# treangenlab/bronko

Measured on AMD Instinct MI355X. Metric: reads/sec through call k-mer->pileup, SARS-CoV-2 k=21, higher is better.
Workload: dtype u64

## Files before the change

### bronko_amd/csrc/bk_engine.cpp

```cpp
#include <hip/hip_runtime.h>

#include <algorithm>
#include <cstdarg>
#include <cstdio>
#include <cstdlib>
#include <cstring>
#include <memory>
#include <string>
#include <vector>

#include "../host/lcb.hpp"
#include "bk_engine.h"

thread_local std::string g_err;

int fail(int code, const char* fmt, ...) {
    char buf[1024];
    va_list ap;
    va_start(ap, fmt);
    vsnprintf(buf, sizeof buf, fmt, ap);
    va_end(ap);
    g_err = buf;
    return code;
}
// ... 430 lines not shown
        int share = ix.n_cus - ix.n_cus / 4;
        if (const char* fr = test_env("BK_ITEM_SHARE")) share = std::max(1, std::min(ix.n_cus, ix.n_cus * atoi(fr) / 16));
        grid = bk::items_grid(take, ix.family.load() > 1 ? share : ix.n_cus);
        if (const char* gr = test_env("BK_ITEM_GRID")) grid = std::max<uint32_t>(1, std::min<uint32_t>(grid, (uint32_t)atoi(gr)));
    }
    return take;
}
static int make_l2_room(bk_engine* e, bk::ScanArgs& a, uint64_t l2_cap) {
    if (e->l2_bits.n < a.n_records * a.l2_words || e->l2_diag.n < a.n_records) {
        BK_HIP(hipStreamSynchronize(e->stream));
        const uint64_t recs = std::min<uint64_t>(std::max<uint64_t>(a.n_records + a.n_records / 4, 1 << 16), l2_cap);
        BK_HIP(e->l2_bits.alloc((size_t)recs * a.l2_words)); BK_HIP(e->n_bits.alloc((size_t)recs * a.l2_words)); BK_HIP(e->l2_diag.alloc((size_t)recs));
        BK_HIP(e->l2_any.alloc((size_t)(recs + 31) / 32)); BK_HIP(e->n_any.alloc((size_t)(recs + 31) / 32));
        for (DevBuf<unsigned int>* b : {&e->l2_bits, &e->l2_any, &e->n_bits, &e->n_any}) BK_HIP(hipMemsetAsync(b->p, 0, b->n * sizeof(unsigned int), e->stream));
    }
    a.l2_bits = e->l2_bits.p; a.l2_diag = e->l2_diag.p; a.l2_any = e->l2_any.p; a.n_bits = e->n_bits.p; a.n_any = e->n_any.p;
    return BK_OK;
}
static int bin_items(bk_engine* e, bk::ScanArgs& a, int mate, uint32_t grid, bool wait_v) {
    const IndexTables& ix = *e->ix;
    MatePlane& pl = e->mate[mate];
    bk_engine::Span sp(e, 3);
    bk::BinArgs b{};
    b.ig = e->ig; b.items = e->items.p; b.tab = e->item_tab.p; b.gext = e->item_gext.p; b.n_wg = grid; b.ov = e->ov.p; b.ov_n = e->ov_n.p; b.ov_cap = (uint32_t)e->ov.n;
    b.ov_par = e->ov_par; e->ov_par ^= 1u;
    b.id_at = ix.id_at.p; b.cell_codes = ix.cell_codes.p + bk::scan_ref_pad_words(); b.win_lo = a.win_lo; b.win_dev = a.win_dev; b.total_cells = (uint32_t)ix.total_cells;
    b.counters = pl.counters.p; b.v_off = ix.v_off; b.v_real_len = bk::v_real_len(ix.n_full, ix.v_span); b.rl = (uint32_t)ix.v_span + 1u;
    const bool v_clean = pl.take_v_clean();
    b.v_mode = ix.item_v_mode >= 0 ? ix.item_v_mode : (v_clean ? 2 : 1);
    if (const char* ba = test_env("BK_BIN_ABLATE")) b.ablate = atoi(ba);
    if (wait_v) {
        e->pending.on = true; e->pending.mate = mate; e->pending.b = b;
        b.part = 1;
        a.touch_v = pl.fuse_touch.p; a.rl_recip = ~0ull / (unsigned long long)(ix.v_span + 1) + 1ull;
        pl.items_wait();
    } else {
        pl.no_more_waiting();
        if (e->fuse_ok) a.touch_v = nullptr;
    }
    BK_HIP(bk::launch_bin_count(b, e->stream));
    return BK_OK;
}
static int level2_and_fold(bk_engine* e, const bk::ScanArgs& a, int mate, uint32_t grid) {
    const IndexTables& ix = *e->ix;
    bk_engine::Span sp(e, 3);
    if (int rc = l2_count_report(e, a)) return rc;
    if (ix.ablate == 1 || ix.ablate == 4) {
        BK_HIP(hipMemsetAsync(e->n_bits.p, 0, (size_t)a.n_records * a.l2_words * sizeof(unsigned int), e->stream));
        BK_HIP(hipMemsetAsync(e->n_any.p, 0, e->n_any.n * sizeof(unsigned int), e->stream));
    }
    else BK_HIP(bk::launch_level2(a, ix.n_cus, e->stream));
    if (!e->use_items) {
        bk::FoldArgs f{};
        f.slabs = e->slabs.p; f.n_slabs = grid; f.n_lds_bins = ix.n_lds_bins; f.id_at = ix.id_at.p; f.cell_codes = ix.cell_codes.p + bk::scan_ref_pad_words(); f.win_lo = a.win_lo; f.win_dev = a.win_dev; f.touch_e = a.touch_e;
        f.counters = e->mate[mate].counters.p;
        bk::launch_fold(f, e->stream);
    }
    return BK_OK;
}
static int push_device(bk_engine* e, int mate, const uint32_t* d_words, uint32_t stride_words, const uint16_t* d_lens, uint64_t n,
                       const unsigned long long* n_records_dev = nullptr, uint64_t kmers_upper = 0) {
    MatePlane& pl = e->mate[mate];
    if (int rc = pl.zero_if_stale(e)) return rc;
    const uint64_t upper = kmers_upper ? kmers_upper : n * (uint64_t)stride_words * 16;
    if (int rc = ensure_ktab_room(e, upper)) return rc;
    if (e->dump) { if (int rc = dump_push(e, mate, d_words, stride_words, d_lens, n, n_records_dev, upper)) return rc; }
    pl.written();
    if (int rc = l2_stats_arm(e)) return rc;
    bk::ScanArgs a = scan_args(e, mate, d_words, stride_words, d_lens, n, n_records_dev);
    if (e->ix->W <= 0) {
        bk::launch_count_kmers(a, e->stream);
    } else {
        if (int rc = choose_window(e, a, n)) return rc;
        const uint64_t l2_cap = std::max<uint64_t>(64, ((1ull << 30) / sizeof(unsigned int)) / a.l2_words);
        for (uint64_t base = 0; base < n; base += a.n_records) {
            uint32_t grid = 0;
            a.rec_base = base; a.n_records = next_launch(e, n - base, l2_cap, grid);
            if (int rc = make_l2_room(e, a, l2_cap)) return rc;
            if (int rc = flush_pending_items(e)) return rc;
            const bool wait_v = e->fuse_ok && a.n_direct && !pl.fuse_off && e->ix->item_v_mode < 0;
            a.l2_plan = e->use_items && e->ix->n_files == 1 && e->ix->family.load() >= 4 && !test_env("BK_NO_L2_PLAN") ? e->l2_plan.p : nullptr;
            {
                bk_engine::Span sp(e, 0);
                if (e->use_items) { a.ov_par = e->ov_par; BK_HIP(bk::launch_scan_items(a, grid, e->stream)); }
                else BK_HIP(bk::launch_scan_count(a, grid, e->stream));
            }
            if (e->use_items) { if (int rc = bin_items(e, a, mate, grid, wait_v)) return rc; }
            if (int rc = level2_and_fold(e, a, mate, grid)) return rc;
        }
    }
    BK_HIP(hipGetLastError());
    if (!n_records_dev) pl.pushed_records += n;
    return note_ktab_fill(e);
}

static constexpr int kPush = 1;
static int push_checks(bk_engine* e, int mate, uint64_t n, bool batch_ok, const char* bad_batch, bool too_large) {
    if (!e) return fail(BK_ERR_INVALID, "null engine");
    if (!e->in_sample) return fail(BK_ERR_STATE, "bk_push_reads_* called before bk_sample_begin");
    if (mate < 0 || mate > 1) return fail(BK_ERR_INVALID, "mate must be 0 or 1");
    if (n == 0) return BK_OK;
    if (!batch_ok) return fail(BK_ERR_INVALID, "%s", bad_batch);
    if (too_large) return fail(BK_ERR_INVALID, "batch too large: push at most 2^32 bases per call");
    BK_HIP(hipSetDevice(e->device));
    return kPush;
}
static int packed_checks(bk_engine* e, int mate, const void* words, uint32_t stride_words, const void* lens, uint64_t n) {
    return push_checks(e, mate, n, words && lens && stride_words != 0 && stride_words <= 4096, "bad record batch",
                       stride_words != 0 && n > (1ull << 32) / ((uint64_t)stride_words * 16));
}
struct PackGeom {
    uint32_t stride; uint64_t cap;
    PackGeom(int k, uint64_t n_reads, uint64_t total, uint64_t longest)
        : stride((uint32_t)std::min<uint64_t>((std::max<uint64_t>(longest, (uint64_t)k) + 15) / 16, 4095)),
          cap(n_reads + total / (uint64_t)k + total / (std::min<uint64_t>((uint64_t)stride * 16, 65535) - (uint64_t)(k - 1)) + 16) {}
};
static int pack_and_push(bk_engine* e, int mate, bk_engine::IngestSlot& sl, const uint8_t* bases, uint32_t shift, const unsigned long long* offsets,
                         uint64_t n_reads, uint64_t total, PackGeom g, const bk::QualArgs* q = nullptr) {
    bk::PackArgs pa{};
    pa.shift = shift; pa.bases = bases; pa.offsets = offsets; pa.n_reads = n_reads; pa.k = e->ix->k; pa.stride_words = g.stride;
    pa.words = sl.d_words.p; pa.lens = sl.d_lens.p; pa.cap = g.cap; pa.n_records = sl.d_nrec.p; pa.work = sl.d_work.p;
    { bk_engine::Span sp(e, 2); bk::launch_pack_reads(pa, e->kstats.p + mate * 4 + 0, e->stream, q); }
    return push_device(e, mate, sl.d_words.p, g.stride, sl.d_lens.p, g.cap, sl.d_nrec.p, total);
}

static constexpr int kMaxMinQual = 93;

static int push_ascii(bk_engine* e, int mate, const uint8_t* buf, const uint8_t* qual, const uint64_t* offsets, uint64_t n_reads, uint32_t thr) {
    const bool too_large = buf && offsets && n_reads && offsets[n_reads] - offsets[0] >= (1ull << 32);
    if (int rc = push_checks(e, mate, n_reads, buf && offsets, "bad read batch", too_large); rc != kPush) return rc;
    const uint64_t base0 = offsets[0], total = offsets[n_reads] - base0;
    if (!e->copy_stream) BK_HIP(hipStreamCreateWithFlags(&e->copy_stream, hipStreamNonBlocking));
    bk_engine::IngestSlot& sl = e->slots[e->next_slot];
    e->next_slot = (e->next_slot + 1) % 3;
    if (!sl.done) { BK_HIP(hipEventCreateWithFlags(&sl.done, hipEventDisableTiming)); BK_HIP(hipEventCreateWithFlags(&sl.uploaded, hipEventDisableTiming)); }
    if (sl.busy) { BK_HIP(hipEventSynchronize(sl.done)); sl.busy = false; }

    if (sl.h_bases_cap < total + 1) {
        if (sl.h_bases) BK_HIP(hipHostFree(sl.h_bases));
        sl.h_bases_cap = total + total / 4 + 4096;
        BK_HIP(hipHostMalloc(reinterpret_cast<void**>(&sl.h_bases), sl.h_bases_cap, hipHostMallocDefault));
    }
    if (sl.h_off_cap < n_reads + 1) {
        if (sl.h_off) BK_HIP(hipHostFree(sl.h_off));
        sl.h_off_cap = n_reads + n_reads / 4 + 1024;
        BK_HIP(hipHostMalloc(reinterpret_cast<void**>(&sl.h_off), sl.h_off_cap * sizeof(unsigned long long), hipHostMallocDefault));
    }
    if (qual && sl.h_quals_cap < total + 1) {
        if (sl.h_quals) BK_HIP(hipHostFree(sl.h_quals));
        sl.h_quals_cap = total + total / 4 + 4096;
        BK_HIP(hipHostMalloc(reinterpret_cast<void**>(&sl.h_quals), sl.h_quals_cap, hipHostMallocDefault));
    }
    std::memcpy(sl.h_bases, buf + base0, total);
    if (qual) std::memcpy(sl.h_quals, qual + base0, total);
    uint64_t longest = 0;
    for (uint64_t i = 0; i <= n_reads; i++) {
        sl.h_off[i] = offsets[i] - base0;
        if (i) longest = std::max(longest, offsets[i] - offsets[i - 1]);
    }
    const PackGeom g(e->ix->k, n_reads, total, longest);

    if (sl.d_bases.n < total + 1) BK_HIP(sl.d_bases.alloc(total + total / 4 + 4096));
    if (qual && sl.d_quals.n < total + 1) BK_HIP(sl.d_quals.alloc(total + total / 4 + 4096));
    if (sl.d_off.n < n_reads + 1) BK_HIP(sl.d_off.alloc(n_reads + n_reads / 4 + 1024));
    if (sl.d_words.n < g.cap * g.stride) BK_HIP(sl.d_words.alloc(g.cap * g.stride + g.cap * g.stride / 4));
    if (sl.d_lens.n < g.cap) BK_HIP(sl.d_lens.alloc(g.cap + g.cap / 4));
    if (!sl.d_nrec.p) BK_HIP(sl.d_nrec.alloc(4));
// ... 725 lines not shown
```

### bronko_amd/csrc/bk_kernels.h

```cpp
#pragma once
#include <hip/hip_runtime.h>

#include "../../include/bronko_hip.h"
#include "bk_device.h"

namespace bk {

struct ItemGeom {
    uint32_t n_ebins, n_vbins;
    uint32_t cap_e, cap_v;
    uint32_t vq_log2;
    uint32_t wg_items;
    uint32_t wg_stride;
    uint32_t grid_max;
};
constexpr uint32_t kEBinLog2 = 7;
constexpr uint32_t kERunMax = 255;
constexpr uint32_t kEBinSpan = (1u << kEBinLog2) + kERunMax;
constexpr uint32_t kItemGCap = 256;

struct ScanArgs {
    const IndexView* ixp;
    int32_t k, wstart, W, v_omin, v_span;
    uint64_t v_off;
    uint32_t total_cells, n_u;
    const uint32_t* ref_words;
    const uint32_t* cell_codes;
    const uint32_t* cell_has;
    const uint32_t* cell_clean;
    const uint32_t* cell_clean3;
    const uint32_t* cell_yf;
    const uint32_t* cell_yr;
    const uint32_t* id_at;
    const uint32_t* cell_fast;
    const uint2* cell_blk;
    const uint32_t* cell_nat;
    const uint32_t* cell_natrow;
    const uint2* seed_tab;
    uint32_t seed_log2;
    const uint2* seed_tab2;
    uint32_t seed2_log2;
    const uint32_t* rc_words;
    const uint32_t* words;
    const uint16_t* lens;
    uint64_t rec_base;
    uint64_t n_records;
    const unsigned long long* n_records_dev;
    uint32_t stride_words;
    unsigned long long* counters;
    unsigned int* slabs;
    unsigned int* n_bits;
    unsigned int* n_any;
    unsigned int* l2_bits;
    unsigned int* l2_any;
    unsigned int* l2_plan;
    uint32_t l2_min_grid;
    uint2* l2_diag;
    uint32_t l2_words;
    uint32_t n_lds_bins;
    uint32_t win_lo;
    const uint32_t* win_dev;
    const uint32_t* occ;
    int32_t win_file, n_files;
    int ref_in_lds;
    unsigned long long* kmer_total;
    unsigned long long* ktab_keys;
    unsigned int* ktab_cnt;
    uint32_t ktab_log2;
    unsigned long long* ktab_overflow;
    uint32_t mate;
    unsigned int* touch_v;
    unsigned int* touch_b;
    unsigned int* touch_p;
    unsigned int* touch_e;
    unsigned long long rl_recip;
    ItemGeom ig;
    unsigned short* items;
    unsigned short* tab;
    unsigned short* gext;
    unsigned int* ov;
    unsigned long long* ov_n;
    uint32_t ov_cap;
    uint32_t ov_par;
    int n_direct;
    uint32_t stage_off;
    int ablate;
    unsigned long long* dbg;
};

struct FinalizeArgs {
    IndexView ix;
    const unsigned long long* counters;
    uint64_t elem_lo, elem_hi;
    unsigned long long ci, cs, cx;
    unsigned long long* pileup;
    size_t plane;
    unsigned long long* stats;
    unsigned char* present;
    unsigned long long* kept_total;
    unsigned long long* distinct_total;
    unsigned int* partials;
    int row_exact, row_general;
    const uint32_t* file_cell_lo;
    uint32_t max_file_cells;
    unsigned int* deferred;
    unsigned long long* deferred_n;
    int clear_v;
    unsigned int* deferred_mask;
    unsigned int* n_deferred;
    unsigned long long* ktab_keys;
    unsigned int* ktab_cnt;
    uint32_t ktab_log2;
    unsigned long long* ktab_overflow;
    uint32_t mate;
    const unsigned int* v_list;
    const unsigned int* p_list;
    const unsigned int* e_list;
    const unsigned int* n_list;
    int mode;
    const int* sel;
    int sel_file;
    unsigned int* lean_e_list;
    unsigned int* lean_n_list;
    int no_lean;
    const unsigned int* tail_e_list;
    const unsigned int* tail_n_list;
    unsigned long long* zero_e;
    size_t zero_e_n;
    int gather;
    int gather_ablate;
    unsigned long long* alias_hits;
    unsigned int* n_alias_hits;
    unsigned int alias_cap;
    const uint64_t* merged_slots;
    uint32_t n_merged_slots;
    const unsigned short* f_items;
    const unsigned short* f_tab;
    const unsigned short* f_gext;
    const unsigned int* f_ov;
    const unsigned long long* f_ov_n;
    uint32_t f_ov_cap, f_ov_par, f_n_wg;
    ItemGeom f_ig;
    unsigned int* f_touch;
};

struct FoldArgs {
    const unsigned int* slabs;
    uint32_t n_slabs;
    uint32_t n_lds_bins;
    const uint32_t* id_at;
    uint32_t win_lo;
    const uint32_t* win_dev;
    unsigned int* touch_e;
    const uint32_t* cell_codes;
    unsigned long long* counters;
};

struct PackArgs {
    const uint8_t* bases;
    uint32_t shift;
    const unsigned long long* offsets;
    uint64_t n_reads;
    int32_t k;
    uint32_t stride_words;
    uint32_t* words;
    uint16_t* lens;
    uint64_t cap;
// ... 145 lines not shown
```

### bronko_amd/csrc/bk_scan_items.hip

```cpp
#include <hip/hip_runtime.h>

#include <algorithm>
#include <mutex>
#include <utility>
#include <vector>

#include "bk_device.h"
#include "bk_kernels.h"
#include "bk_scan_common.h"

namespace bk {

constexpr int kItemBlock = 1024;
constexpr int kItemWaves = kItemBlock / 64;
constexpr int kItemGroupsPerCu = 1;
constexpr uint32_t kListCap = 256;
constexpr uint32_t kListWords = kListCap + 4u;
constexpr uint32_t kDealRing = 32;
constexpr size_t kItemLdsFixed = (4 + 4 + 2 * kDealRing + kItemWaves * kListWords) * sizeof(unsigned int);
constexpr int kBinBlock = 256;
constexpr uint32_t kMaxChunkMismatches = 24;
constexpr uint32_t kStageMaxWords = 12;

__device__ __forceinline__ void item_direct(const __attribute__((address_space(4))) ScanArgs* ap, uint32_t bin, uint32_t item, uint32_t win_lo) {
    const __attribute__((address_space(4))) ScanArgs& a = *ap;
    if (bin < a.ig.n_ebins) {
        const uint32_t c0 = win_lo + (bin << kEBinLog2) + (item & 127u), n = ((item >> 7) & 255u) + 1u, rev = item >> 15;
        for (uint32_t i = 0; i < n; ++i) {
            const uint32_t cell = c0 + i;
            const uint32_t id = a.id_at[cell];
            const uint32_t rc = ((a.cell_codes[kRefPadWords + (cell >> 4)] >> (2u * (cell & 15u))) & 3u) == 2u ? 1u : 0u;
            atomicAdd(a.counters + 2 * (size_t)id + (rc ^ rev), 1ull);
        }
    } else {
        const uint64_t at = (uint64_t)(bin - a.ig.n_ebins) * ((6ull << a.ig.vq_log2) * (uint32_t)(a.v_span + 1)) + (item & 0x7fffu);
        atomicAdd(a.counters + a.v_off + at, (item & 0x8000u) ? ~0ull : 1ull);
    }
}

template <int KT, bool STAGED>
__global__ __launch_bounds__(kItemBlock) void scan_items_kernel(ScanArgs a) {
    extern __shared__ __attribute__((aligned(16))) unsigned char smem[];
    unsigned int* block_kmers = reinterpret_cast<unsigned int*>(smem);
    unsigned int* wg_ctr = block_kmers + 4;
    uint2* ring = reinterpret_cast<uint2*>(wg_ctr + 4);
    unsigned int* lst_all = wg_ctr + 4 + 2 * kDealRing;
    unsigned int* cnt = lst_all + kItemWaves * kListWords;
    const uint32_t n_eb = a.ig.n_ebins, n_bins = n_eb + a.ig.n_vbins, cap_e = a.ig.cap_e, cap_v = a.ig.cap_v;
    const uint32_t nb_pad = (n_bins + 3u) & ~3u;
    unsigned short* buck = reinterpret_cast<unsigned short*>(cnt + nb_pad);
    unsigned int* lds_ref = reinterpret_cast<unsigned int*>(smem + ((kItemLdsFixed + (size_t)nb_pad * 4u + (size_t)a.ig.wg_stride * 2u + 7u) & ~(size_t)7u));

    const int lane = threadIdx.x & 63;
    const int wave = __builtin_amdgcn_readfirstlane((int)(threadIdx.x >> 6));
    unsigned int* const lst = lst_all + (uint32_t)wave * kListWords;
    typedef const __attribute__((address_space(4))) ScanArgs* ColdArgs;
    const ColdArgs cold0 = (ColdArgs)__builtin_amdgcn_kernarg_segment_ptr();
    auto cold = [&]() __attribute__((always_inline)) -> ColdArgs { ColdArgs p = cold0; asm volatile("" : "+s"(p)); return p; };

    asm volatile("v_mov_b32 v127, 0" ::: "v127");
    BK_DBG_CLOCK(a, 0);
    const uint32_t total = a.total_cells;
    const uint32_t win_lo = a.win_dev ? a.win_dev[1] : a.win_lo;
    const uint32_t win_file = a.win_dev ? a.win_dev[0] : (uint32_t)a.win_file;
    const uint32_t lds_cells = min(total - win_lo, a.n_lds_bins);
    const uint32_t n_refw = kRefPadWords + (lds_cells + 15) / 16 + kRefBackWords;
    const uint32_t n_bitw = kBitPadWords + (lds_cells + 31) / 32 + kBitBackWords;
    const uint32_t n_blk = (lds_cells + 63) / 64 + 2;
    const uint32_t blk_w0 = (n_refw + 2u * n_bitw + 1u) & ~1u;
    const uint32_t rc_lo = total - win_lo - lds_cells, rc_base = rc_lo & 15u;
    const uint32_t rc_w0 = blk_w0 + 2u * n_blk;
    uint64_t n_records = a.n_records;
    if (a.n_records_dev) {
        const uint64_t nd = *a.n_records_dev;
        n_records = nd > a.rec_base ? min(nd - a.rec_base, a.n_records) : 0ull;
    }
    const uint32_t* const words0 = a.words + a.rec_base * a.stride_words;
    const uint16_t* const lens0 = a.lens + a.rec_base;
    const uint64_t n_tiles = (n_records + 63) / 64;
    unsigned int* const deal_ctr = reinterpret_cast<unsigned int*>(cold()->ov_n + 2);
    const uint64_t t_hi = n_tiles;
    const uint32_t sw = a.stride_words;
    unsigned int* const rec_buf = reinterpret_cast<unsigned int*>(smem + a.stage_off) + (uint32_t)wave * 64u * sw;
    auto stage = [&](uint64_t t) -> uint32_t {
        if (t >= t_hi) return 0u;
        const uint64_t rr = t * 64 + (uint32_t)lane;
        const uint32_t ln = rr < n_records ? (uint32_t)lens0[rr] : 0u;
        if ((t + 1) * 64 <= n_records) {
            const unsigned char* g = reinterpret_cast<const unsigned char*>(words0 + t * 64 * sw);
            unsigned char* l = reinterpret_cast<unsigned char*>(rec_buf);
            for (uint32_t u0 = 0; u0 < 16u * sw; u0 += 64u) {
                const uint32_t u = u0 + (uint32_t)lane;
                if (u < 16u * sw)
                    __builtin_amdgcn_global_load_lds((const __attribute__((address_space(1))) void*)(g + (size_t)u * 16u),
                                                     (__attribute__((address_space(3))) void*)(l + (size_t)u0 * 16u), 16, 0, 0);
            }
        } else if (rr < n_records) {
            const uint32_t* src = words0 + rr * sw;
            for (uint32_t j = 0; j < sw; ++j) rec_buf[(uint32_t)lane * sw + j] = src[j];
        }
        return ln;
    };
    uint32_t len_pf = 0u;
    const uint64_t tile0 = (uint64_t)blockIdx.x * kItemWaves + (uint32_t)wave;
    if constexpr (STAGED) len_pf = stage(tile0);
    BK_DBG_CLOCK2(a, 0);
    uint32_t chunk1 = 0u;
    if (threadIdx.x == 0) {
        const uint32_t par = cold()->ov_par;
        if (blockIdx.x == 0) deal_ctr[par ^ 1u] = 0u;
        chunk1 = gridDim.x + __hip_atomic_fetch_add(deal_ctr + par, 1u, __ATOMIC_RELAXED, __HIP_MEMORY_SCOPE_AGENT);
    }

    for (uint32_t i = threadIdx.x; i < n_bins; i += kItemBlock) cnt[i] = 0u;
    if (lane == 0) lst[0] = 0u;
    if (threadIdx.x == 0) wg_ctr[1] = (unsigned int)kItemWaves;
    {
        const ColdArgs c = cold();
        const uint32_t* const g_ref = c->ref_words + (win_lo >> 4);
        const uint32_t* const g_fast = c->cell_fast + (win_lo >> 5);
        const uint32_t* const g_c3 = c->cell_clean3 + (win_lo >> 5);
        const uint32_t* const g_blk = reinterpret_cast<const uint32_t*>(c->cell_blk + (win_lo >> 6));
        const uint32_t* const g_rc = c->rc_words + (rc_lo >> 4);
        const uint32_t c0 = n_refw, c1 = c0 + n_bitw, c2 = c1 + n_bitw, c3 = c2 + 2u * n_blk, c4 = c3 + n_refw + 1u;
        for (uint32_t b0 = 0; b0 < c4; b0 += 8u * kItemBlock) {
            uint32_t v[8];
#pragma unroll
            for (uint32_t u = 0; u < 8u; ++u) {
                const uint32_t i = b0 + u * kItemBlock + threadIdx.x;
                const uint32_t* src = i < c0 ? g_ref + i : i < c1 ? g_fast + (i - c0) : i < c2 ? g_c3 + (i - c1) : i < c3 ? g_blk + (i - c2) : g_rc + (i - c3);
                v[u] = i < c4 ? *src : 0u;
            }
#pragma unroll
            for (uint32_t u = 0; u < 8u; ++u) {
                const uint32_t i = b0 + u * kItemBlock + threadIdx.x;
                if (i < c4) lds_ref[i < c2 ? i : i < c3 ? blk_w0 + (i - c2) : rc_w0 + (i - c3)] = v[u];
            }
        }
    }
    BK_DBG_CLOCK2(a, 1);
    if (threadIdx.x == 0) { ring[0] = make_uint2(0u, blockIdx.x); ring[1] = make_uint2(1u, chunk1); }
    __syncthreads();
    BK_DBG_CLOCK(a, 1);
    const unsigned int* refw1 = lds_ref + kRefPadWords;
    const unsigned int* fastw = lds_ref + n_refw + kBitPadWords;
    const unsigned int* c3w = lds_ref + n_refw + n_bitw + kBitPadWords;
    const uint2* blkw = reinterpret_cast<const uint2*>(lds_ref + blk_w0);
    const int32_t rc_sym0 = (int32_t)(rc_w0 * 16u);

    const int k = KT ? KT : a.k;
    const uint64_t kmask = (1ull << (2 * k)) - 1ull;
    const uint32_t km1 = (uint32_t)k - 1u;
    const int omin = a.v_omin, span = a.v_span;
    const uint32_t rl = (uint32_t)span + 1u, vq_log2 = a.ig.vq_log2, vqm = (1u << vq_log2) - 1u;
    const uint32_t v_buck0 = n_eb * cap_e;
    const uint32_t last_word = a.stride_words - 1u;

    auto put_ext = [&](uint32_t bin, uint32_t g , uint32_t item) {
        const ColdArgs c = cold();
        if (g < kItemGCap) { c->gext[((size_t)blockIdx.x * n_bins + bin) * kItemGCap + g] = (unsigned short)item; return; }
        const unsigned long long i = atomicAdd(c->ov_n + c->ov_par, 1ull);
        if (i < (unsigned long long)c->ov_cap) c->ov[i] = (bin << 16) | item;
        else item_direct(c, bin, item, win_lo);
    };
    auto emit_e = [&](bool on, uint32_t c_lo, uint32_t n, bool f) {
        uint32_t c = c_lo, left = (on && !BK_ABLATE(a, 14)) ? n : 0u;
        do {
            const uint32_t take = min(left, kERunMax);
            if (left) {
                const uint32_t bin = c >> kEBinLog2;
                const uint32_t item = (c & 127u) | ((take - 1u) << 7) | (f ? 0u : 0x8000u);
                const uint32_t s = __hip_atomic_fetch_add(&cnt[bin], 1u, __ATOMIC_RELAXED, __HIP_MEMORY_SCOPE_WORKGROUP);
                if (s < cap_e) buck[bin * cap_e + s] = (unsigned short)item; else put_ext(bin, s - cap_e, item);
            }
            c += take; left -= take;
        } while (__ballot(left != 0u));
    };

    uint32_t nkm = 0;
    auto n_mark = [&](bool on, uint32_t rec, uint32_t sk, uint32_t n, int32_t dgm, uint32_t flm) {
        if (!on) return;
        const ColdArgs c = cold();
        unsigned int* row = c->n_bits + (size_t)rec * c->l2_words;
        atomicOr(c->n_any + (rec >> 5), 1u << (rec & 31u));
        c->l2_diag[rec] = make_uint2((uint32_t)dgm, flm);
        uint32_t w = sk >> 5, bit = sk & 31u, left = n;
        while (left) {
            const uint32_t take = min(left, 32u - bit);
            atomicOr(row + w, (take == 32u ? 0xffffffffu : (1u << take) - 1u) << bit);
            left -= take; ++w; bit = 0u;
        }
    };
    auto l2_mark = [&](bool on, uint32_t rec, uint32_t sk, uint32_t n, int32_t dgm, uint32_t flm) {
        if (!on) return;
        const ColdArgs c = cold();
        unsigned int* row = c->l2_bits + (size_t)rec * c->l2_words;
        atomicOr(c->l2_any + (rec >> 5), 1u << (rec & 31u));
        c->l2_diag[rec] = make_uint2((uint32_t)dgm, flm);
        uint32_t w = sk >> 5, bit = sk & 31u, left = n;
        while (left) {
            const uint32_t take = min(left, 32u - bit);
            atomicOr(row + w, (take == 32u ? 0xffffffffu : (1u << take) - 1u) << bit);
            left -= take; ++w; bit = 0u;
        }
    };
    const bool stats = a.ktab_keys != nullptr;

    auto take_tile = [&]() __attribute__((always_inline)) -> uint64_t {
        uint32_t t = 0u;
        if (lane == 0) {
            const uint32_t s = __hip_atomic_fetch_add(wg_ctr + 1, 1u, __ATOMIC_RELAXED, __HIP_MEMORY_SCOPE_WORKGROUP);
            const uint32_t q = s / kItemWaves, i = s % kItemWaves;
            volatile uint2* const rg = ring;
            if (i == 0u) {
                const uint32_t cn = gridDim.x + __hip_atomic_fetch_add(deal_ctr + cold()->ov_par, 1u, __ATOMIC_RELAXED, __HIP_MEMORY_SCOPE_AGENT);
                rg[(q + 1u) % kDealRing].y = cn;
                __builtin_amdgcn_fence(__ATOMIC_RELEASE, "workgroup");
                rg[(q + 1u) % kDealRing].x = q + 1u;
            }
            while (rg[q % kDealRing].x != q) __builtin_amdgcn_s_sleep(1);
            __builtin_amdgcn_fence(__ATOMIC_ACQUIRE, "workgroup");
            t = rg[q % kDealRing].y * kItemWaves + i;
        }
        return (uint64_t)(uint32_t)__builtin_amdgcn_readfirstlane((int)t);
    };
    uint32_t pf_sink = 0;
    const uint2* const seed_tab = a.seed_tab2 ? a.seed_tab2 + ((size_t)win_file << a.seed2_log2) : nullptr;
    const uint32_t hint_len = n_records ? (uint32_t)__builtin_amdgcn_readfirstlane((int)lens0[0]) : 0u;
    const uint32_t hint_span = hint_len >= (uint32_t)k ? hint_len - (uint32_t)k : 0u;
    const uint32_t um_sh = 64u - 2u * km1;
    const uint32_t um8 = um_sh >= 32u ? 0u : 0xffffffffu << um_sh, um9 = um_sh >= 32u ? 0xffffffffu << (um_sh - 32u) : 0xffffffffu;

    struct SeedSet { uint64_t g[3]; uint32_t h[3]; uint2 b[3]; };
    auto seed_pos = [&](int sround, int j) __attribute__((always_inline)) -> uint32_t {
        const int qj = sround ? kSeeds - 2 : (j == 0 ? 0 : j == 1 ? kSeeds - 1 : 1);
        return (hint_span * (uint32_t)qj) / (uint32_t)(kSeeds - 1);
    };
    auto seed_load = [&](const uint32_t* __restrict__ wr, int sround, int ns, SeedSet& S) __attribute__((always_inline)) {
#pragma unroll
        for (int j = 0; j < 3; ++j) {
            if (j >= ns) continue;
            S.g[j] = read_symbols_at(wr, seed_pos(sround, j), last_word) & kmask;
            S.h[j] = seed_hash(S.g[j]);
            S.b[j] = seed_tab[S.h[j] >> (32u - a.seed2_log2)];
        }
    };
    const bool use_tab = seed_tab && !BK_ABLATE(a, 9) && !BK_ABLATE(a, 11);

    for (uint64_t tile = tile0, next_tile = 0; tile < t_hi; tile = next_tile) {
        const uint64_t r = tile * 64 + lane;
        next_tile = take_tile();
        const bool live = r < n_records;
        const uint32_t r32 = live ? (uint32_t)r : 0u;
        uint32_t len;
        if constexpr (STAGED) {
            asm volatile("s_waitcnt vmcnt(0) lgkmcnt(0)" ::: "memory");
            len = len_pf;
        } else {
            len = live ? (uint32_t)lens0[r32] : 0u;
        }
        if (len < (uint32_t)k) len = 0u;
        if (tile == tile0) BK_DBG_CLOCK2(a, 2);
        const uint32_t maxlen = wave_max(len);
        const uint32_t* __restrict__ w = STAGED ? rec_buf + (uint32_t)lane * sw : words0 + (uint64_t)r32 * a.stride_words;
        const uint32_t nk = len ? len - km1 : 0u;
        nkm += nk;
        if constexpr (!STAGED) {
            const uint64_t nt = next_tile;
            const uint64_t first = nt * 64ull * a.stride_words, words_tile = 64ull * a.stride_words;
            const uint64_t at = first + (uint64_t)lane * 32ull;
            if (nt < t_hi && (uint64_t)lane * 32ull < words_tile && at < n_records * a.stride_words)
                asm volatile("global_load_dword %0, %1, off" : "=v"(pf_sink) : "v"(words0 + at) : "memory");
        }
        SeedSet S;
        if (use_tab && maxlen) seed_load(w, 0, 3, S);
        bool next_sent = false;
        auto send_next = [&]() __attribute__((always_inline)) {
            if constexpr (STAGED) { if (!next_sent) { asm volatile("s_waitcnt lgkmcnt(0)" ::: "memory"); len_pf = stage(next_tile); next_sent = true; } }
        };
        auto ask_next = [&]() __attribute__((always_inline)) { send_next(); };
        if (!maxlen) { ask_next(); continue; }

        bool fwd = true, seeded = false, l1ok = false;
        int32_t dg = 0;
        auto accept = [&](bool hit, int32_t d0, bool f) __attribute__((always_inline)) {
            const int32_t span_k = (int32_t)(len - (uint32_t)k);
            const int32_t lo_cell = f ? d0 : d0 - span_k;
            const int32_t hi_cell = f ? d0 + span_k : d0;
            const bool ok = hit && len != 0u && lo_cell >= 0 && (uint32_t)hi_cell + (uint32_t)k <= total;
            const bool inw = ok && (uint32_t)lo_cell >= win_lo && (uint32_t)hi_cell < win_lo + a.n_lds_bins;
            const uint32_t tail = blkw[inw ? ((uint32_t)lo_cell >> 6) - (win_lo >> 6) : 0u].y;
            dg = ok ? d0 : dg; fwd = ok ? f : fwd; seeded = seeded || ok;
            l1ok = ok ? (inw && (uint32_t)hi_cell < tail) : l1ok;
        };
        for (int sround = 0; sround < 2 && use_tab; ++sround) {
            if (sround == 1) {
                if (!__ballot(len != 0u && !seeded)) break;
                seed_load(w, 1, 1, S);
            }
            const int ns = sround ? 1 : 3;
            bool hit = false, hf = true;
            int32_t hd0 = 0;
#pragma unroll
            for (int j = 2; j >= 0; --j) {
                if (j >= ns) continue;
                const uint32_t s = seed_pos(sround, j);
                const uint32_t tag = S.h[j] & 15u;
                const uint64_t sg = S.g[j];
                const uint32_t ent = (S.b[j].x != 0xffffffffu && (S.b[j].x >> 28) == tag) ? S.b[j].x : S.b[j].y;
                const uint32_t cell = ent & ((1u << kSeedCellBits) - 1u), strand = (ent >> kSeedCellBits) & 1u;
                const bool in_ref = !seeded && ent != 0xffffffffu && (ent >> 28) == tag && s + (uint32_t)k <= len &&
// ... 413 lines not shown
        const uint32_t win_lo = b.win_dev ? b.win_dev[1] : b.win_lo;
        for (uint32_t i = threadIdx.x; i < kEBinSpan && !BK_ABLATE(b, 2) && !BK_ABLATE(b, 3); i += kBinBlock) {
            const uint32_t s0 = acc[i], s1 = acc[(kEBinSpan + 1u) + i];
            if (s0 | s1) {
                const uint32_t cell = win_lo + (bin << kEBinLog2) + i;
                const uint32_t id = b.id_at[cell];
                const uint32_t rc = ((b.cell_codes[cell >> 4] >> (2u * (cell & 15u))) & 3u) == 2u ? 1u : 0u;
                if (s0) atomicAdd(b.counters + 2 * (size_t)id + rc, (unsigned long long)s0);
                if (s1) atomicAdd(b.counters + 2 * (size_t)id + (1u - rc), (unsigned long long)s1);
            }
        }
    } else {
        const uint64_t first = (uint64_t)(bin - n_eb) * vsize;
        unsigned long long* const vc = b.counters + b.v_off + first;
        const uint32_t n_here = (uint32_t)min((uint64_t)vsize, b.v_real_len > first ? b.v_real_len - first : 0ull);
        if (BK_ABLATE(b, 2) || BK_ABLATE(b, 4)) {
        } else if (b.v_mode == 2 && b.ov_n[b.ov_par] <= (unsigned long long)b.ov_cap) {
            for (uint32_t i = threadIdx.x; i < n_here; i += kBinBlock) vc[i] = (unsigned long long)(long long)(int32_t)acc[i];
        } else if (b.v_mode == 1 || b.v_mode == 2) {
            for (uint32_t i = threadIdx.x; i < n_here; i += kBinBlock) vc[i] += (unsigned long long)(long long)(int32_t)acc[i];
        } else {
            for (uint32_t i = threadIdx.x; i < n_here; i += kBinBlock) {
                const uint32_t v = acc[i];
                if (v) atomicAdd(vc + i, (unsigned long long)(long long)(int32_t)v);
            }
        }
    }
}

bool item_geometry(uint32_t win_cells, uint32_t n_full, int v_span, ItemGeom* g) {
    if (v_span <= 0 || win_cells == 0 || n_full == 0) return false;
    const uint32_t rl = (uint32_t)v_span + 1u;
    const uint64_t n_q = (uint64_t)n_full + (uint32_t)v_span;
    uint32_t vq_log2 = 0, nv = 0;
    for (uint32_t l = 6; l <= 8; ++l) {
        if ((6u << l) * rl > 32767u) break;
        vq_log2 = l;
        nv = (uint32_t)((n_q + (1u << l) - 1u) >> l);
        if (nv <= 512u) break;
    }
    if (!vq_log2 || nv > 1024u) return false;
    const uint32_t ne = (win_cells + (1u << kEBinLog2) - 1u) >> kEBinLog2;
    if (ne + nv > 2u * (uint32_t)kItemBlock) return false;
    g->n_ebins = ne; g->n_vbins = nv; g->vq_log2 = vq_log2;
    g->cap_e = 48u; g->cap_v = 24u;
    g->wg_items = ne * g->cap_e + nv * g->cap_v;
    g->wg_stride = g->wg_items;
    g->grid_max = 0;
    return true;
}

uint32_t items_max_grid(int n_cus) { return (uint32_t)n_cus * kItemGroupsPerCu; }
uint32_t items_grid(uint64_t n_records, int n_cus) {
    const uint64_t tiles = (n_records + 63) / 64;
    const uint64_t want = (tiles + kItemWaves - 1) / kItemWaves;
    return (uint32_t)std::max<uint64_t>(1, std::min<uint64_t>(want, items_max_grid(n_cus)));
}
size_t items_lds_bytes(const ItemGeom& g, uint32_t win_cells) {
    const size_t nb_pad = ((size_t)g.n_ebins + g.n_vbins + 3u) & ~(size_t)3u;
    return ((kItemLdsFixed + nb_pad * 4u + (size_t)g.wg_stride * 2u + 7u) & ~(size_t)7u) + scan_ref_lds_bytes(win_cells) + 8u +
           ((size_t)(kRefPadWords + (win_cells + 15) / 16 + kRefBackWords) + 1u) * sizeof(unsigned int);
}

hipError_t raise_lds_limit(const void* fn, size_t lds) {
    static std::mutex mu;
    static std::vector<std::pair<std::pair<const void*, int>, size_t>> have;
    int dev = 0;
    (void)hipGetDevice(&dev);
    std::lock_guard<std::mutex> lock(mu);
    size_t* cur = nullptr;
    for (auto& h : have) if (h.first.first == fn && h.first.second == dev) cur = &h.second;
    if (!cur || *cur < lds) {
        hipError_t e = hipFuncSetAttribute(fn, hipFuncAttributeMaxDynamicSharedMemorySize, (int)lds);
        if (e != hipSuccess) return e;
        if (cur) *cur = lds; else have.push_back({{fn, dev}, lds});
    }
    return hipSuccess;
}

hipError_t launch_scan_items(const ScanArgs& a, uint32_t grid, hipStream_t stream) {
    if (a.n_records == 0 || a.W <= 0) return hipSuccess;
    size_t lds = items_lds_bytes(a.ig, std::min(a.n_lds_bins, a.total_cells));
    ScanArgs b = a;
    const uintptr_t first = reinterpret_cast<uintptr_t>(a.words + a.rec_base * a.stride_words);
    const size_t stage_off = (lds + 15u) & ~(size_t)15u, stage_end = stage_off + (size_t)kItemWaves * 64u * a.stride_words * sizeof(unsigned int) + 128u;
    const bool staged = a.stride_words <= kStageMaxWords && (first & 15u) == 0 && stage_end <= 160u * 1024u && !BK_ABLATE(a, 16);
    b.stage_off = 0;
    if (staged) {
        b.stage_off = (uint32_t)stage_off;
        lds = stage_end;
    }
    void (*kern)(ScanArgs);
    if (staged) kern = a.k == 21 ? scan_items_kernel<21, true> : a.k == 31 ? scan_items_kernel<31, true> : scan_items_kernel<0, true>;
    else kern = a.k == 21 ? scan_items_kernel<21, false> : a.k == 31 ? scan_items_kernel<31, false> : scan_items_kernel<0, false>;
    if (hipError_t e = raise_lds_limit(reinterpret_cast<const void*>(kern), lds)) return e;
    hipLaunchKernelGGL(kern, dim3(grid), dim3(kItemBlock), lds, stream, b);
    return hipGetLastError();
}

hipError_t launch_bin_count(const BinArgs& b, hipStream_t stream) {
    const uint32_t n_bins = b.part == 1 ? b.ig.n_ebins : b.part == 2 ? b.ig.n_vbins : b.ig.n_ebins + b.ig.n_vbins;
    if (n_bins == 0 || b.n_wg == 0) return hipSuccess;
    const size_t lds = std::max<size_t>(2u * (kEBinSpan + 1u), (size_t)(6u << b.ig.vq_log2) * b.rl) * sizeof(unsigned int);
    if (hipError_t e = raise_lds_limit(reinterpret_cast<const void*>(bin_count_kernel), lds)) return e;
    hipLaunchKernelGGL(bin_count_kernel, dim3(n_bins), dim3(kBinBlock), lds, stream, b);
    return hipGetLastError();
}

}
```

Before: 8.669 billion.

## Deal tail tiles in smaller pieces to balance work across workgroups

Changes the dynamic tile dealing in the item scan kernel so that the first chunks go out as full 16-tile groups and the final chunks are handed out in smaller pieces (8 tiles by default, configurable through BK_DEAL). The goal is to cut tail imbalance, where a few workgroups finish large chunks late while the rest sit idle. The ring-based take_tile loop now decodes the piece size from the high bits of the chunk entry and has waves skip slots beyond the piece. This costs more global atomics and ring handoffs near the end of each launch.

```diff
diff --git a/bronko_amd/csrc/bk_engine.cpp b/bronko_amd/csrc/bk_engine.cpp
--- a/bronko_amd/csrc/bk_engine.cpp
+++ b/bronko_amd/csrc/bk_engine.cpp
@@ -536,7 +536,14 @@
             a.l2_plan = e->use_items && e->ix->n_files == 1 && e->ix->family.load() >= 4 && !test_env("BK_NO_L2_PLAN") ? e->l2_plan.p : nullptr;
             {
                 bk_engine::Span sp(e, 0);
-                if (e->use_items) { a.ov_par = e->ov_par; BK_HIP(bk::launch_scan_items(a, grid, e->stream)); }
+                if (e->use_items) {
+                    a.ov_par = e->ov_par;
+                    if (const char* dl = test_env("BK_DEAL")) {
+                        unsigned f = 16, p = 4;
+                        if (sscanf(dl, "%u,%u", &f, &p) == 2 && (p == 1 || p == 2 || p == 4 || p == 8 || p == 16)) { a.deal_fine = (uint32_t)((uint64_t)grid * f / 16); a.deal_piece = p; }
+                    }
+                    BK_HIP(bk::launch_scan_items(a, grid, e->stream));
+                }
                 else BK_HIP(bk::launch_scan_count(a, grid, e->stream));
             }
             if (e->use_items) { if (int rc = bin_items(e, a, mate, grid, wait_v)) return rc; }
diff --git a/bronko_amd/csrc/bk_kernels.h b/bronko_amd/csrc/bk_kernels.h
--- a/bronko_amd/csrc/bk_kernels.h
+++ b/bronko_amd/csrc/bk_kernels.h
@@ -83,6 +83,7 @@
     uint32_t ov_cap;
     uint32_t ov_par;
     int n_direct;
+    uint32_t deal_fine, deal_piece;
     uint32_t stage_off;
     int ablate;
     unsigned long long* dbg;
diff --git a/bronko_amd/csrc/bk_scan_items.hip b/bronko_amd/csrc/bk_scan_items.hip
--- a/bronko_amd/csrc/bk_scan_items.hip
+++ b/bronko_amd/csrc/bk_scan_items.hip
@@ -80,6 +80,15 @@
     const uint64_t n_tiles = (n_records + 63) / 64;
     unsigned int* const deal_ctr = reinterpret_cast<unsigned int*>(cold()->ov_n + 2);
     const uint64_t t_hi = n_tiles;
+    auto deal_piece = [&](uint32_t d) __attribute__((always_inline)) -> uint32_t {
+        const ColdArgs c = cold();
+        const uint32_t nt = (uint32_t)t_hi, n_chunks = (nt + (uint32_t)kItemWaves - 1u) / (uint32_t)kItemWaves;
+        const uint32_t fine = c->deal_fine, piece = c->deal_piece;
+        const uint32_t F = max((uint32_t)gridDim.x, n_chunks > fine ? n_chunks - fine : 0u);
+        if (d < F) return min(d * (uint32_t)kItemWaves, nt) | ((uint32_t)(kItemWaves - 1) << 28);
+        const uint64_t first = (uint64_t)F * kItemWaves + (uint64_t)(d - F) * piece;
+        return (uint32_t)min(first, (uint64_t)nt) | ((piece - 1u) << 28);
+    };
     const uint32_t sw = a.stride_words;
     unsigned int* const rec_buf = reinterpret_cast<unsigned int*>(smem + a.stage_off) + (uint32_t)wave * 64u * sw;
     auto stage = [&](uint64_t t) -> uint32_t {
@@ -104,17 +113,19 @@
     uint32_t len_pf = 0u;
     const uint64_t tile0 = (uint64_t)blockIdx.x * kItemWaves + (uint32_t)wave;
     if constexpr (STAGED) len_pf = stage(tile0);
+    const uint32_t hint_raw = n_records ? (uint32_t)lens0[0] : 0u;
     BK_DBG_CLOCK2(a, 0);
     uint32_t chunk1 = 0u;
     if (threadIdx.x == 0) {
         const uint32_t par = cold()->ov_par;
         if (blockIdx.x == 0) deal_ctr[par ^ 1u] = 0u;
-        chunk1 = gridDim.x + __hip_atomic_fetch_add(deal_ctr + par, 1u, __ATOMIC_RELAXED, __HIP_MEMORY_SCOPE_AGENT);
+        chunk1 = deal_piece(gridDim.x + __hip_atomic_fetch_add(deal_ctr + par, 1u, __ATOMIC_RELAXED, __HIP_MEMORY_SCOPE_AGENT));
     }
 
     for (uint32_t i = threadIdx.x; i < n_bins; i += kItemBlock) cnt[i] = 0u;
     if (lane == 0) lst[0] = 0u;
     if (threadIdx.x == 0) wg_ctr[1] = (unsigned int)kItemWaves;
+    if (threadIdx.x >= 2u && threadIdx.x < kDealRing) ring[threadIdx.x].x = 0xffffffffu;
     {
         const ColdArgs c = cold();
         const uint32_t* const g_ref = c->ref_words + (win_lo >> 4);
@@ -139,7 +150,7 @@
         }
     }
     BK_DBG_CLOCK2(a, 1);
-    if (threadIdx.x == 0) { ring[0] = make_uint2(0u, blockIdx.x); ring[1] = make_uint2(1u, chunk1); }
+    if (threadIdx.x == 0) { ring[0] = make_uint2(0u, deal_piece(blockIdx.x)); ring[1] = make_uint2(1u, chunk1); }
     __syncthreads();
     BK_DBG_CLOCK(a, 1);
     const unsigned int* refw1 = lds_ref + kRefPadWords;
@@ -209,24 +220,28 @@
     auto take_tile = [&]() __attribute__((always_inline)) -> uint64_t {
         uint32_t t = 0u;
         if (lane == 0) {
-            const uint32_t s = __hip_atomic_fetch_add(wg_ctr + 1, 1u, __ATOMIC_RELAXED, __HIP_MEMORY_SCOPE_WORKGROUP);
-            const uint32_t q = s / kItemWaves, i = s % kItemWaves;
             volatile uint2* const rg = ring;
-            if (i == 0u) {
-                const uint32_t cn = gridDim.x + __hip_atomic_fetch_add(deal_ctr + cold()->ov_par, 1u, __ATOMIC_RELAXED, __HIP_MEMORY_SCOPE_AGENT);
-                rg[(q + 1u) % kDealRing].y = cn;
-                __builtin_amdgcn_fence(__ATOMIC_RELEASE, "workgroup");
-                rg[(q + 1u) % kDealRing].x = q + 1u;
-            }
-            while (rg[q % kDealRing].x != q) __builtin_amdgcn_s_sleep(1);
-            __builtin_amdgcn_fence(__ATOMIC_ACQUIRE, "workgroup");
-            t = rg[q % kDealRing].y * kItemWaves + i;
+            for (;;) {
+                const uint32_t s = __hip_atomic_fetch_add(wg_ctr + 1, 1u, __ATOMIC_RELAXED, __HIP_MEMORY_SCOPE_WORKGROUP);
+                const uint32_t q = s / kItemWaves, i = s % kItemWaves;
+                while (rg[q % kDealRing].x != q) __builtin_amdgcn_s_sleep(1);
+                __builtin_amdgcn_fence(__ATOMIC_ACQUIRE, "workgroup");
+                const uint32_t p = rg[q % kDealRing].y, first = p & 0x0fffffffu;
+                if (i == 0u) {
+                    const uint32_t pn = deal_piece(gridDim.x + __hip_atomic_fetch_add(deal_ctr + cold()->ov_par, 1u, __ATOMIC_RELAXED, __HIP_MEMORY_SCOPE_AGENT));
+                    rg[(q + 1u) % kDealRing].y = pn;
+                    __builtin_amdgcn_fence(__ATOMIC_RELEASE, "workgroup");
+                    rg[(q + 1u) % kDealRing].x = q + 1u;
+                }
+                t = min(first + i, (uint32_t)t_hi);
+                if (i <= (p >> 28) || first >= (uint32_t)t_hi) break;
+            }
         }
         return (uint64_t)(uint32_t)__builtin_amdgcn_readfirstlane((int)t);
     };
     uint32_t pf_sink = 0;
     const uint2* const seed_tab = a.seed_tab2 ? a.seed_tab2 + ((size_t)win_file << a.seed2_log2) : nullptr;
-    const uint32_t hint_len = n_records ? (uint32_t)__builtin_amdgcn_readfirstlane((int)lens0[0]) : 0u;
+    const uint32_t hint_len = (uint32_t)__builtin_amdgcn_readfirstlane((int)hint_raw);
     const uint32_t hint_span = hint_len >= (uint32_t)k ? hint_len - (uint32_t)k : 0u;
     const uint32_t um_sh = 64u - 2u * km1;
     const uint32_t um8 = um_sh >= 32u ? 0u : 0xffffffffu << um_sh, um9 = um_sh >= 32u ? 0xffffffffu << (um_sh - 32u) : 0xffffffffu;
@@ -806,6 +821,7 @@
     if (a.n_records == 0 || a.W <= 0) return hipSuccess;
     size_t lds = items_lds_bytes(a.ig, std::min(a.n_lds_bins, a.total_cells));
     ScanArgs b = a;
+    if (!b.deal_piece) { b.deal_piece = 8u; b.deal_fine = grid; }
     const uintptr_t first = reinterpret_cast<uintptr_t>(a.words + a.rec_base * a.stride_words);
     const size_t stage_off = (lds + 15u) & ~(size_t)15u, stage_end = stage_off + (size_t)kItemWaves * 64u * a.stride_words * sizeof(unsigned int) + 128u;
     const bool staged = a.stride_words <= kStageMaxWords && (first & 15u) == 0 && stage_end <= 160u * 1024u && !BK_ABLATE(a, 16);
```

Measured after the change: 8.708 billion, median of 6. No clear change (+0.4%).
